# ScissorJack-ever/AlayaLite

Hardware: AMD Instinct MI355X
Metric: QPS @ recall@10>=0.95, GIST-960 L2, 1M base / 1k queries (higher is better)
Workload: dtype f32

## Files before the change

alayalite_amd/csrc/capi.cpp:

```cpp
#include "../../include/alaya_hip.h"

#include <hip/hip_runtime_api.h>

#include <algorithm>
#include <cfloat>
#include <cmath>
#include <cstring>
#include <memory>
#include <mutex>
#include <stdexcept>
#include <limits>
#include <string>
#include <thread>
#include <vector>

#include "build_kernels.h"
#include "extend_kernels.h"
#include "graph_update.h"
#include "hnsw_build.h"
#include "flat_bound.h"
#include "flat_filtered_kernels.h"
#include "flat_kernels.h"
#include <cstdlib>
#include "screen_bound.h"
// ... 93 lines not shown
  bool norms_ready = false;
  DevBuf flat_tiles, tiles_cand, tiles_qexp;
  bool tiles_ready = false;
  int tiles_exp = 0;
  int tiles_metric = -1;
  float max_norm = 0.f;
  DevBuf work, overflow, dirty, stab, q_buf, id_buf, dist_buf, cnt_buf, dlist_buf, dout_buf;
  DevBuf allow_buf, group_buf;
  DevBuf through_buf;
  DevBuf ff_ids, ff_sums, ff_count, ff_part_d, ff_part_i, ff_qlist;
  uint64_t ff_last[4] = {0, 0, 0, 0};
  size_t overflow_clean = 0;
  size_t stab_clean = 0;
  uint32_t hash_log2_override = 0;
  int helpers_mode = -1;
  DevBuf help_stats;
  uint64_t help_stats_slots = 0;
  struct ScreenCopy {
    DevBuf rows, err;
    uint64_t cap = 0;
    bool ready = false;
    bool failed = false;
  };
  ScreenCopy screen_copy[2];
  uint32_t screen_format = 0;
  DevBuf screen_stats;
  uint64_t screen_stats_slots = 0;
  uint32_t last_grid = 0, last_waves = 0;
  uint32_t last_lds = 0, last_hash_log2 = 0, last_compact = 0, last_per_cu = 0, last_scout = 0;
  DevBuf scout_stats;
  uint64_t scout_stats_slots = 0;
  DevBuf scout_policy_stats;
  uint32_t last_scout_policy = 0;
  int visited_mode_override = 0;
  int num_cus = 0;
  uint64_t capacity = 0;
  std::unique_ptr<alaya_amd::HostGraph> upd_graph;
  std::unique_ptr<alaya_amd::RowMirror> upd_rows;
  std::unique_ptr<alaya_amd::UpdateContext> upd_ctx;
  hipStream_t stream = nullptr;
  hipEvent_t scratch_ev = nullptr;
  hipStream_t scratch_stream = nullptr;
  bool scratch_used = false;
  uint64_t device_bytes() const {
    return base.bytes + valid.bytes + l0.bytes + levels.bytes + upper_off.bytes +
           upper_edges.bytes + eps.bytes + overflow.bytes + dirty.bytes + stab.bytes + codes.bytes + sq_min.bytes +
           sq_max.bytes;
  }
};

namespace {

void set_device(const alaya_index *ix) { hip_check(hipSetDevice(ix->device), "hipSetDevice"); }

void scratch_acquire(alaya_index *ix, hipStream_t s) {
  if (ix->scratch_used && ix->scratch_stream != s)
    hip_check(hipStreamWaitEvent(s, ix->scratch_ev, 0), "hipStreamWaitEvent");
}
void scratch_release(alaya_index *ix, hipStream_t s) {
  hip_check(hipEventRecord(ix->scratch_ev, s), "hipEventRecord");
  ix->scratch_stream = s;
  ix->scratch_used = true;
}
void scratch_suspect(alaya_index *ix) {
  ix->overflow_clean = 0;
  ix->stab_clean = 0;
// ... 225 lines not shown

struct SearchPlan {
  const alaya_amd::SearchVariant *variant;
  int W;
  size_t lds;
  int grid;
  int per_cu;
};

uint32_t scout_default(uint32_t dim) { return (dim == 768 || dim == 960) ? alaya_amd::kScoutOn : 0u; }

uint32_t scout_requested(uint32_t dim) {
  const char *e = std::getenv("ALAYA_SEARCH_SCOUT");
  const int asked = e && e[0] ? std::atoi(e) : -1;
  uint32_t f = asked < 0 ? scout_default(dim) : (asked == 1 ? alaya_amd::kScoutOn : (asked == 2 ? alaya_amd::kScoutOn | alaya_amd::kScoutVerify : 0u));
  if (f != 0u) {
    const char *m = std::getenv("ALAYA_SEARCH_SCOUT_MISS");
    if (m && std::atoi(m) != 0) f |= alaya_amd::kScoutMiss;
  }
  return f;
}

uint32_t scout_policy_default(uint32_t dim) {
  return (dim == 768 || dim == 960) ? (alaya_amd::kScoutEarly | alaya_amd::kScoutRecheck) : 0u;
}

uint32_t scout_policy_requested(uint32_t dim) {
  const char *e = std::getenv("ALAYA_SEARCH_SCOUT_POLICY");
  if (!(e && e[0])) return scout_policy_default(dim);
  return static_cast<uint32_t>(std::strtoul(e, nullptr, 0)) &
         (alaya_amd::kScoutEarly | alaya_amd::kScoutRecheck);
}

SearchPlan plan_search(alaya_index *ix, SearchParams &p, alaya_amd::SearchRequest r, uint64_t nq, uint32_t ef,
                       hipStream_t stream) {
  using namespace alaya_amd;
  SearchPlan plan{};
  for (;;) {
    plan.variant = &resolve_search_variant(r);
    const int mode = plan.variant->mode;
    if ((r.want & kModeStamp) != 0 && (mode & kModeStamp) == 0)
      throw ArgError("no stamped search kernel for dim " + std::to_string(ix->dim) +
                     (p.sq8_order ? " SQ8 (order " + std::to_string(p.sq8_order) + ")" : std::string(" f32")) +
                     ": see the variant list in search_variants.h");
    p.help = (mode & kModeHelp) != 0;
    p.two_waves = (mode & kModeTwoWaves) != 0;
    p.screen = (mode & kModeScreen) != 0 ? ix->screen_format : 0u;
    plan.W = p.help ? 4 : search_waves(p);
    while (!p.help && plan.W > 1 && static_cast<uint64_t>(plan.W) > nq) plan.W /= 2;
    p.hash_log2 = size_visited(ix, p, *plan.variant, nq, ef, plan.W);
    const bool compact = p.vis_rbits != kVisWide;
    p.wave_lds = static_cast<uint32_t>(search_wave_lds_bytes(ix->stride, ef, p.hash_log2, compact, p.sq8_order));
    bool fits = true;
    if (p.help) {
      const size_t need = static_cast<size_t>(plan.W) * kHelpMemoSlots * ix->R * 8;
      const size_t q_bytes = search_query_lds_bytes(ix->stride, p.sq8_order);
      if (q_bytes >= need) {
        p.memo_off = 0;
      } else if (p.wave_lds >= q_bytes + 3 * 64 * 4 + need) {
        p.memo_off = static_cast<uint32_t>(q_bytes + 3 * 64 * 4);
      } else {
        fits = false;
      }
    }
    plan.lds = search_shared_lds_bytes(ix->stride, p.sq8_order != 0) + static_cast<size_t>(plan.W) * p.wave_lds +
               (p.help ? kHelpBoardBytes : 0);
    if (!p.help || (fits && plan.lds <= kLdsPerCu)) break;
    r.want &= ~kModeHelp;
  }
  if (plan.lds > kLdsPerCu) throw ArgError("ef / dim too large for the LDS budget");
  int per_cu = 0;
  hip_check(search_occupancy(*plan.variant, p.ip, plan.W, plan.lds, &per_cu), "occupancy");
  per_cu = static_cast<int>(std::max<uint64_t>(1, std::min<uint64_t>(per_cu, max_search_waves_per_cu() / plan.W)));
  const uint64_t cus = static_cast<uint64_t>(stream_cus(ix, stream));
  const uint64_t blocks_needed = p.help ? static_cast<uint64_t>(per_cu) * cus : (nq + plan.W - 1) / plan.W;
  plan.grid = static_cast<int>(std::max<uint64_t>(1, std::min<uint64_t>(blocks_needed, static_cast<uint64_t>(per_cu) * cus)));
  plan.per_cu = per_cu;
  p.scout = 0u;
  p.scout_policy = 0u;
  const uint32_t scout = scout_requested(ix->dim);
  if (scout != 0u && p.screen == 3u && !p.ip && !p.two_waves && !p.help && plan.W == 1 && ix->R <= kScoutR &&
      (plan.variant->mode & ~kModeScreen) == 0 && search_has_two_waves(ix->dim, p.sq8_order, ix->generic) &&
      !helpers_requested(ix, p, nq, cus)) {
    SearchRequest r2 = r;
    r2.want |= kModeTwoWaves;
    const SearchVariant &v2 = resolve_search_variant(r2);
    const size_t lds2 = plan.lds + kScoutBoardBytes;
    int per_cu2 = 0;
    if (v2.mode == (kModeScreen | kModeTwoWaves) && lds2 <= kLdsPerCu)
      hip_check(search_occupancy(v2, false, 2, lds2, &per_cu2), "occupancy");
    if (per_cu2 >= per_cu && nq <= static_cast<uint64_t>(per_cu) * cus) {
      plan.variant = &v2;
      plan.lds = lds2;
      p.scout = scout;
      p.scout_policy = scout_policy_requested(ix->dim);
      if (const char *e = std::getenv("ALAYA_SEARCH_SCOUT_GRID"))
        plan.grid = std::max(1, std::min(plan.grid, std::atoi(e)));
    }
  }
  return plan;
}

SearchParams graph_search_params(alaya_index *ix, const float *d_q, uint64_t nq, uint32_t k, uint32_t ef, uint32_t *d_ids,
                                 float *d_dists, uint32_t *d_cnt) {
  SearchParams p = base_params(ix);
  p.l0 = ix->l0.as<uint32_t>();
  p.R = ix->R;
  p.dedup_edges = ix->dedup;
  p.levels = ix->has_overlay ? ix->levels.as<uint32_t>() : nullptr;
  p.upper_off = ix->upper_off.as<uint64_t>();
  p.upper_edges = ix->upper_edges.as<uint32_t>();
  p.upper_R = ix->upper_R;
  p.ep = ix->ep;
  p.eps = ix->eps.as<uint32_t>();
  p.n_eps = ix->n_eps;
  p.queries = d_q;
  p.nq = nq;
  p.q_stride = ix->dim;
  p.k = k;
  p.ef = ef;
  p.out_ids = d_ids;
  p.out_dists = d_dists;
  p.out_counters = d_cnt;
  return p;
}

void set_search_space(alaya_index *ix, SearchParams &p, bool sq8, uint32_t ef) {
  if (sq8) {
    p.sq8_order = ix->sq8_order;
    p.codes = ix->codes.as<uint8_t>();
    p.code_stride = ix->code_stride;
    p.sq_min = ix->sq_min.as<float>();
    p.sq_max = ix->sq_max.as<float>();
  }
  p.stab_log2 = spill_table_log2(p.sq8_order, std::max<uint32_t>(1, ceil_log2(std::max<uint64_t>(ix->n, 2))), ef);
}

void record_launch(alaya_index *ix, SearchParams &p, int grid, int wg_waves, size_t lds, int per_cu, uint64_t searchers,
                   hipStream_t stream) {
  ix->last_grid = static_cast<uint32_t>(grid);
  ix->last_waves = static_cast<uint32_t>(wg_waves);
  ix->last_lds = static_cast<uint32_t>(lds);
  ix->last_hash_log2 = p.hash_log2;
  ix->last_compact = p.vis_rbits != alaya_amd::kVisWide ? 1u : 0u;
  ix->last_per_cu = static_cast<uint32_t>(per_cu);
  ix->last_scout = p.scout;
  ix->last_scout_policy = p.scout_policy;
  ix->scout_stats_slots = p.scout ? searchers : 0;
  ix->help_stats_slots = p.help ? searchers : 0;
  ix->screen_stats_slots = p.screen ? searchers : 0;
  ix->work.reserve(4);
  p.work_counter = ix->work.as<uint32_t>();
  hip_check(hipMemsetAsync(p.work_counter, 0, 4, stream), "hipMemsetAsync");
}

void do_search(alaya_index *ix, const float *d_q, uint64_t nq, uint32_t k, uint32_t ef,
               uint32_t *d_ids, float *d_dists, uint32_t *d_cnt, hipStream_t stream,
               uint64_t *d_stamps = nullptr, bool sq8 = false, uint32_t fill_id = 0) {
  if (!ix->base.ptr) throw ArgError("index has no base vectors");
  if (!ix->has_graph) throw ArgError("index has no graph");
  if (ef == 0) throw ArgError("ef must be >= 1");
  if (k == 0 || nq == 0) return;
  if (ix->graph_n > ix->n) throw ArgError("graph has more nodes than base vectors");
  SearchParams p = graph_search_params(ix, d_q, nq, k, ef, d_ids, d_dists, d_cnt);
  p.stamps = d_stamps;
  p.fill_id = fill_id;
  if (sq8 && !ix->has_sq8) throw ArgError("index has no SQ8 codes");
  set_search_space(ix, p, sq8, ef);
  if (const char *e = std::getenv("ALAYA_HELP_FLAGS")) p.help_flags = static_cast<uint32_t>(std::strtoul(e, nullptr, 10));
  const SearchPlan plan = plan_search(ix, p, search_request(ix, p, nq, ef, stream), nq, ef, stream);
  if (p.screen >= 2) {
    p.screen_u8 = ix->screen_copy[1].rows.as<uint8_t>();
  } else if (p.screen) {
    p.screen_rows = ix->screen_copy[0].rows.as<uint16_t>();
    p.screen_err = ix->screen_copy[0].err.as<float>();
  }
  scratch_acquire(ix, stream);
  const uint64_t searchers = static_cast<uint64_t>(plan.grid) * plan.W;
  prepare_spill(ix, p, searchers, stream);
  const int wg_waves = p.scout ? 2 * plan.W : plan.W;
  if (p.scout) {
    ix->scout_stats.reserve(searchers * 16);
    p.scout_stats = ix->scout_stats.as<uint32_t>();
    ix->scout_policy_stats.reserve(searchers * 12);
    p.scout_policy_stats = ix->scout_policy_stats.as<uint32_t>();
  }
// ... 1982 lines not shown
    hipStream_t s = nullptr;
    hip_check(hipExtStreamCreateWithCUMask(&s, static_cast<uint32_t>(mask.size()), mask.data()),
              "hipExtStreamCreateWithCUMask");
    *stream = s;
  });
}

int alaya_stream_destroy(void *stream) {
  return guarded([&] {
    if (stream) hip_check(hipStreamDestroy(static_cast<hipStream_t>(stream)), "hipStreamDestroy");
  });
}

int alaya_index_last_launch(const alaya_index *ix, uint32_t *workgroups, uint32_t *waves_per_group) {
  return guarded([&] {
    if (!ix) throw ArgError("null index");
    if (workgroups) *workgroups = ix->last_grid;
    if (waves_per_group) *waves_per_group = ix->last_waves;
  });
}

int alaya_index_last_plan(const alaya_index *ix, uint32_t *lds_bytes, uint32_t *hash_log2, uint32_t *compact,
                          uint32_t *groups_per_cu, uint32_t *scout) {
  return guarded([&] {
    if (!ix) throw ArgError("null index");
    if (lds_bytes) *lds_bytes = ix->last_lds;
    if (hash_log2) *hash_log2 = ix->last_hash_log2;
    if (compact) *compact = ix->last_compact;
    if (groups_per_cu) *groups_per_cu = ix->last_per_cu;
    if (scout) *scout = ix->last_scout;
  });
}

static std::vector<uint64_t> searcher_stats(alaya_index *ix, const DevBuf &buf, uint64_t searchers, uint32_t words) {
  std::vector<uint64_t> t(words, 0);
  if (searchers) {
    set_device(ix);
    scratch_drain(ix);
    std::vector<uint32_t> h(words * searchers);
    hip_check(hipMemcpy(h.data(), buf.ptr, h.size() * 4, hipMemcpyDeviceToHost), "D2H");
    for (uint64_t i = 0; i < h.size(); ++i) t[i % words] += h[i];
  }
  return t;
}

int alaya_index_scout_stats(alaya_index *ix, uint64_t *expansions, uint64_t *hits, uint64_t *records,
                            uint64_t *mismatches) {
  return guarded_scratch(ix, [&] {
    if (!ix) throw ArgError("null index");
    const std::vector<uint64_t> t = searcher_stats(ix, ix->scout_stats, ix->scout_stats_slots, 4);
    if (expansions) *expansions = t[0];
    if (hits) *hits = t[1];
    if (records) *records = t[2];
    if (mismatches) *mismatches = t[3];
  });
}

int alaya_index_scout_policy_stats(alaya_index *ix, uint32_t *policy, uint64_t *early_posts, uint64_t *confirmed,
                                   uint64_t *abandoned) {
  return guarded_scratch(ix, [&] {
    if (!ix) throw ArgError("null index");
    const bool sums = early_posts || confirmed || abandoned;
    const std::vector<uint64_t> t = searcher_stats(ix, ix->scout_policy_stats, sums ? ix->scout_stats_slots : 0, 3);
    if (policy) *policy = ix->last_scout_policy;
    if (early_posts) *early_posts = t[0];
    if (confirmed) *confirmed = t[1];
    if (abandoned) *abandoned = t[2];
  });
}

int alaya_index_set_helpers(alaya_index *ix, int mode) {
  return guarded([&] {
    if (!ix) throw ArgError("null index");
    if (mode < -1 || mode > 1) throw ArgError("helpers mode must be -1 (automatic), 0 (off) or 1 (on)");
    ix->helpers_mode = mode;
  });
}

int alaya_index_help_stats(alaya_index *ix, uint64_t *memo_dists, uint64_t *memo_expansions, uint64_t *helper_rows) {
  return guarded_scratch(ix, [&] {
    if (!ix) throw ArgError("null index");
    const std::vector<uint64_t> t = searcher_stats(ix, ix->help_stats, ix->help_stats_slots, 3);
    if (memo_dists) *memo_dists = t[0];
    if (memo_expansions) *memo_expansions = t[1];
    if (helper_rows) *helper_rows = t[2];
  });
}

int alaya_screen_lower_bound(const float *d_tilde, const float *e_row, uint64_t n, uint32_t dim, float *out) {
  return guarded([&] {
    if (n && (!d_tilde || !e_row || !out)) throw ArgError("invalid arguments");
    for (uint64_t i = 0; i < n; ++i) out[i] = alaya_amd::screen_lower_bound(d_tilde[i], e_row[i], dim);
  });
}

namespace {
void screen_u8_quantize_one(const float *x, uint32_t dim, uint8_t *codes, float *header, float *values) {
  using namespace alaya_amd;
  float lo = FLT_MAX, hi = -FLT_MAX;
  bool bad = false;
// ... 138 lines not shown
```

alayalite_amd/csrc/pybind_module.cpp:

```cpp
#include <pybind11/numpy.h>
#include <pybind11/pybind11.h>
#include <pybind11/stl.h>

#include <algorithm>
#include <cmath>
#include <cstring>
#include <fstream>
#include <memory>
#include <queue>
#include <stdexcept>
#include <string>
#include <vector>

#include "../../include/alaya_hip.h"

extern "C" int alaya_index_flat_diag(alaya_index *, const float *, uint64_t, uint32_t, int, uint32_t *, float *,
                                     uint32_t *, uint32_t *, void *);
#include "host_distance.h"

namespace py = pybind11;

namespace alaya_py {

enum class IndexType { FLAT = 0, HNSW = 1, NSG = 2, FUSION = 3, QG = 4 };
// ... 112 lines not shown
  void set_hash_log2(uint32_t v) { check(alaya_index_set_hash_log2(ix_, v)); }
  void set_visited_mode(int m) { check(alaya_index_set_visited_mode(ix_, m)); }
  void set_helpers(int m) { check(alaya_index_set_helpers(ix_, m)); }
  py::tuple last_launch() {
    uint32_t g = 0, w = 0;
    check(alaya_index_last_launch(ix_, &g, &w));
    return py::make_tuple(g, w);
  }
  py::tuple help_stats() {
    uint64_t m = 0, x = 0, r = 0;
    check(alaya_index_help_stats(ix_, &m, &x, &r));
    return py::make_tuple(m, x, r);
  }
  py::tuple screen_stats() {
    uint64_t a = 0, b = 0;
    check(alaya_index_screen_stats(ix_, &a, &b));
    return py::make_tuple(a, b);
  }
  py::tuple scout_stats() {
    uint64_t e = 0, h = 0, r = 0, m = 0;
    check(alaya_index_scout_stats(ix_, &e, &h, &r, &m));
    return py::make_tuple(e, h, r, m);
  }
  py::tuple scout_policy_stats() {
    uint64_t a = 0, c = 0, d = 0;
    check(alaya_index_scout_policy_stats(ix_, nullptr, &a, &c, &d));
    return py::make_tuple(a, c, d);
  }
  uint32_t scout_policy() {
    uint32_t pol = 0;
    check(alaya_index_scout_policy_stats(ix_, &pol, nullptr, nullptr, nullptr));
    return pol;
  }
  py::dict last_plan() {
    uint32_t g = 0, w = 0, lds = 0, hl = 0, c = 0, pc = 0, sc = 0;
    check(alaya_index_last_launch(ix_, &g, &w));
    check(alaya_index_last_plan(ix_, &lds, &hl, &c, &pc, &sc));
    py::dict d;
    d["workgroups"] = g;
    d["waves_per_group"] = w;
    d["lds_bytes"] = lds;
    d["hash_log2"] = hl;
    d["compact"] = c != 0;
    d["groups_per_cu"] = pc;
    d["scout"] = sc;
    d["scout_policy"] = scout_policy();
    return d;
  }

 protected:
  alaya_index *ix_ = nullptr;
};

class PyIndexInterface : public LaunchControls {
 public:
  explicit PyIndexInterface(const IndexParams &params) : params_(params) {
    dtype_ = dtype_code(params_.data_type_);
    if (params_.id_type_.is(py::dtype::of<uint32_t>())) {
      id_bytes_ = 4;
    } else if (params_.id_type_.is(py::dtype::of<uint64_t>())) {
      id_bytes_ = 8;
    } else {
      throw std::runtime_error("Unsupported id type");
    }
    if (params_.quantization_type_ == QuantizationType::SQ4 ||
        params_.quantization_type_ == QuantizationType::RABITQ)
      throw std::runtime_error("quantization type not supported by the MI355X engine (SQ4/RaBitQ are out of scope)");
    if (params_.metric_ == MetricType::COS && dtype_ != kF32 && dtype_ != kF64) {
      throw std::runtime_error("COS metric only support float or double");
    }
    if (params_.quantization_type_ == QuantizationType::SQ8 && dtype_ != kF32)
      throw std::runtime_error("SQ8 quantization of non-float32 data is not supported by the MI355X engine");
    check(alaya_index_create(0, &ix_));
  }
  ~PyIndexInterface() {
    if (graph_) alaya_graph_free(graph_);
    if (ix_) alaya_index_destroy(ix_);
  }
  PyIndexInterface(const PyIndexInterface &) = delete;
// ... 958 lines not shown
      .def("get_data_by_id", &PyIndexInterface::get_data_by_id, py::arg("id"))
      .def("insert", &PyIndexInterface::insert, py::arg("insert_data"), py::arg("ef"))
      .def("remove", &PyIndexInterface::remove, py::arg("id"))
      .def("add", &PyIndexInterface::add, py::arg("vectors"), py::arg("ef_construction"))
      .def("sq8_codes", &PyIndexInterface::sq8_codes)
      .def("sq8_range", &PyIndexInterface::sq8_range)
      .def("last_build_device_ms", &PyIndexInterface::last_build_device_ms)
      .def("batch_search", &PyIndexInterface::batch_search, py::arg("queries"), py::arg("topk"),
           py::arg("ef"), py::arg("num_threads"))
      .def("batch_search_with_distance", &PyIndexInterface::batch_search_with_distance,
           py::arg("queries"), py::arg("topk"), py::arg("ef"), py::arg("num_threads"))
      .def("exact_search", &PyIndexInterface::exact_search, py::arg("queries"), py::arg("topk"))
      .def("exact_search_filtered", &PyIndexInterface::exact_search_filtered, py::arg("queries"), py::arg("topk"),
           py::arg("allow_words"), py::arg("mask_of_query") = py::none())
      .def("save", &PyIndexInterface::save, py::arg("index_path"), py::arg("data_path"),
           py::arg("quant_path") = std::string())
      .def("load", &PyIndexInterface::load, py::arg("index_path"), py::arg("data_path"),
           py::arg("quant_path") = std::string())
      .def("filtered_search", &PyIndexInterface::filtered_search, py::arg("queries"), py::arg("topk"), py::arg("ef"),
           py::arg("allow_words"), py::arg("mask_of_query") = py::none(), py::arg("pool") = 0,
           py::arg("through") = false)
      .def("last_through", &PyIndexInterface::last_through)
      .def("get_data_dim", &PyIndexInterface::get_data_dim)
      .def("get_data_num", &PyIndexInterface::get_data_num)
      .def("last_counters", &PyIndexInterface::last_counters)
      .def("set_hash_log2", &PyIndexInterface::set_hash_log2)
      .def("set_visited_mode", &PyIndexInterface::set_visited_mode)
      .def("set_helpers", &PyIndexInterface::set_helpers)
      .def("last_launch", &PyIndexInterface::last_launch)
      .def("help_stats", &PyIndexInterface::help_stats)
      .def("screen_stats", &PyIndexInterface::screen_stats)
      .def("scout_stats", &PyIndexInterface::scout_stats)
      .def("scout_policy_stats", &PyIndexInterface::scout_policy_stats)
      .def("last_plan", &PyIndexInterface::last_plan)
      .def("set_rerank_mode", &PyIndexInterface::set_rerank_mode)
      .def("rerank_mode", &PyIndexInterface::rerank_mode)
      .def("device_distances", &PyIndexInterface::device_distances)
      .def("graph_arrays", &PyIndexInterface::graph_arrays);


  py::class_<Graph, std::shared_ptr<Graph>>(m, "Graph")
      .def_static("build", &Graph::build, py::arg("data"), py::arg("metric") = 0, py::arg("R") = 32u,
                  py::arg("ef_construction") = 100u, py::arg("num_threads") = 1u, py::arg("seed") = 100u)
      .def_static("load", &Graph::load, py::arg("path"), py::arg("id_bytes") = 4)
      .def_static("from_arrays", &Graph::from_arrays, py::arg("l0"), py::arg("levels"), py::arg("upper_off"),
                  py::arg("upper_edges"), py::arg("upper_R"), py::arg("ep"), py::arg("eps") = py::none())
      .def("save", &Graph::save, py::arg("path"), py::arg("id_bytes") = 4, py::arg("capacity") = 0u)
      .def("arrays", &Graph::arrays);
  py::class_<DeviceIndex, std::shared_ptr<DeviceIndex>>(m, "DeviceIndex")
      .def(py::init<int>(), py::arg("device") = 0)
      .def("set_base", &DeviceIndex::set_base, py::arg("rows"), py::arg("metric") = 0, py::arg("valid") = py::none())
      .def("set_graph", &DeviceIndex::set_graph)
      .def("build_graph", &DeviceIndex::build_graph, py::arg("R") = 32, py::arg("ef_construction") = 100,
           py::arg("seed") = 100, py::arg("batch_div") = 0, py::arg("max_batch") = 0, py::arg("refine") = 2)
      .def("extend_graph", &DeviceIndex::extend_graph, py::arg("rows"), py::arg("ef_construction") = 100,
           py::arg("seed") = 100, py::arg("batch_div") = 0, py::arg("max_batch") = 0, py::arg("refine") = 2)
      .def("read_sq8", &DeviceIndex::read_sq8, py::arg("first"), py::arg("count"))
      .def("search", &DeviceIndex::search, py::arg("queries"), py::arg("k"), py::arg("ef"))
      .def("search_device", &DeviceIndex::search_device)
      .def("filtered_search", &DeviceIndex::filtered_search, py::arg("queries"), py::arg("k"), py::arg("ef"),
           py::arg("allow_words"), py::arg("mask_of_query") = py::none())
      .def("filtered_search_device", &DeviceIndex::filtered_search_device)
      .def("filtered_search_hop", &DeviceIndex::filtered_search_hop, py::arg("queries"), py::arg("k"), py::arg("ef"),
           py::arg("allow_words"), py::arg("mask_of_query") = py::none())
      .def("filtered_search_hop_device", &DeviceIndex::filtered_search_hop_device)
      .def("filtered_search_sq8", &DeviceIndex::filtered_search_sq8, py::arg("queries"), py::arg("k"), py::arg("ef"),
           py::arg("allow_words"), py::arg("mask_of_query") = py::none(), py::arg("pool") = 0,
           py::arg("rerank_queries") = py::none())
      .def("filtered_search_sq8_device", &DeviceIndex::filtered_search_sq8_device)
      .def("shard_search_device", &DeviceIndex::shard_search_device)
      .def("distances", &DeviceIndex::distances)
      .def("set_hash_log2", &DeviceIndex::set_hash_log2)
      .def("set_visited_mode", &DeviceIndex::set_visited_mode)
      .def("set_helpers", &DeviceIndex::set_helpers)
      .def("last_launch", &DeviceIndex::last_launch)
      .def("help_stats", &DeviceIndex::help_stats)
      .def("screen_stats", &DeviceIndex::screen_stats)
      .def("scout_stats", &DeviceIndex::scout_stats)
      .def("scout_policy_stats", &DeviceIndex::scout_policy_stats)
      .def("last_plan", &DeviceIndex::last_plan)
      .def("flat_search", &DeviceIndex::flat_search, py::arg("queries"), py::arg("k"))
      .def("flat_search_device", &DeviceIndex::flat_search_device)
      .def("flat_search_filtered", &DeviceIndex::flat_search_filtered, py::arg("queries"), py::arg("k"),
           py::arg("allow_words"), py::arg("mask_of_query") = py::none())
      .def("flat_search_filtered_device", &DeviceIndex::flat_search_filtered_device)
      .def("flat_filtered_last", &DeviceIndex::flat_filtered_last)
      .def("flat_diag", &DeviceIndex::flat_diag)
      .def("flat_contraction", &DeviceIndex::flat_contraction)
      .def("search_sq8_device", &DeviceIndex::search_sq8_device)
      .def("shard_search_sq8_device", &DeviceIndex::shard_search_sq8_device)
      .def("set_sq8", &DeviceIndex::set_sq8, py::arg("codes"), py::arg("min"), py::arg("max"), py::arg("order") = 2)
      .def("search_sq8", &DeviceIndex::search_sq8, py::arg("queries"), py::arg("k"), py::arg("ef"),
           py::arg("rerank") = 1, py::arg("rerank_queries") = py::none())
      .def("profile_search", &DeviceIndex::profile_search, py::arg("q"), py::arg("k"), py::arg("ef"),
           py::arg("space") = 0)
      .def("device_bytes", &DeviceIndex::device_bytes);
  m.def("sq8_train", [](F32Array data) {
    const uint32_t d = static_cast<uint32_t>(data.shape(1));
    py::array_t<float> mn(d), mx(d);
    check(alaya_sq8_train(data.data(), data.shape(0), d, mn.mutable_data(), mx.mutable_data()));
    return py::make_tuple(mn, mx);
  });
  m.def("sq8_encode", [](F32Array data, F32Array mn, F32Array mx, uint32_t threads) {
    py::array_t<uint8_t> codes({data.shape(0), data.shape(1)});
    check(alaya_sq8_encode(data.data(), data.shape(0), static_cast<uint32_t>(data.shape(1)), mn.data(), mx.data(),
                           codes.mutable_data(), threads));
    return codes;
  }, py::arg("data"), py::arg("min"), py::arg("max"), py::arg("num_threads") = 1u);
  m.def("host_sq8_order", &host_sq8_order);
  m.def("build_batches", [](U32Array levels, uint64_t start, uint32_t ep, uint32_t batch_div, uint32_t max_batch) {
    if (levels.ndim() != 1) throw py::value_error("levels must be 1D");
    const uint64_t n = levels.shape(0);
// ... 97 lines not shown
```

alayalite_amd/csrc/search_kernels.h:

```cpp
#pragma once
#include <hip/hip_runtime_api.h>

#include <cstddef>
#include <cstdint>

#include "search_variants.h"

namespace alaya_amd {

struct SearchParams {
  const float *base;
  uint64_t n;
  uint32_t dim;
  uint32_t stride;
  const uint32_t *valid;
  bool ip;
  bool generic;
  const uint32_t *l0;
  uint32_t R;
  bool dedup_edges;
  const uint32_t *levels;
  const uint64_t *upper_off;
  const uint32_t *upper_edges;
  uint32_t upper_R;
// ... 13 lines not shown
  uint32_t *overflow_bits;
  uint32_t *dirty_words;
  uint32_t dirty_cap;
  uint32_t wave_lds;
  uint32_t hash_log2;
  uint32_t vis_rbits;
  uint32_t vis_lbits;
  uint32_t vis_max_disp;
  uint32_t vis_limit;
  uint16_t *spill_table;
  uint32_t stab_log2;
  uint32_t stab_rbits;
  uint32_t spill_flags;
  uint64_t *stamps;
  int sq8_order;
  const uint8_t *codes;
  uint32_t code_stride;
  const float *sq_min;
  const float *sq_max;
  uint32_t help;
  uint32_t help_flags;
  uint32_t memo_off;
  uint32_t two_waves;
  uint32_t *help_stats;
  uint32_t screen;
  const uint16_t *screen_rows;
  const float *screen_err;
  const uint8_t *screen_u8;
  uint32_t *screen_stats;
  uint32_t scout;
  uint32_t *scout_stats;
  uint32_t scout_policy;
  uint32_t *scout_policy_stats;
};
constexpr uint32_t kScoutOn = 1, kScoutVerify = 2, kScoutMiss = 4;
constexpr uint32_t kScoutEarly = 1, kScoutRecheck = 2;
constexpr uint32_t kScoutSlots = 3;
constexpr uint32_t kScoutR = 32;
constexpr size_t kScoutBoardBytes = kScoutSlots * (kScoutR * 4 + 8 + 4) + 20;

struct FilterParams {
  const uint32_t *allow;
  const uint32_t *mask_of_query;
  uint32_t mask_words;
  uint32_t k;
  uint32_t result_off;
};

struct HopParams {
  uint32_t *n_through;
};

struct RerankParams {
  const uint32_t *search_ids;
  uint32_t k;
  uint32_t n_src;
  uint32_t n_take;
  uint32_t zeros;
  uint32_t fill_id;
  uint32_t *out_ids;
  float *out_dists;
};

constexpr uint32_t kVisWide = 0xffffffffu;
constexpr size_t kHelpBoardBytes = 256;
#ifndef ALAYA_HELP_DEPTH
#define ALAYA_HELP_DEPTH 1
#endif
constexpr size_t kHelpMemoSlots = ALAYA_HELP_DEPTH + 1;
constexpr uint32_t kStabBucket = 8;
inline size_t visited_table_bytes(uint32_t hash_log2, bool compact) {
// ... 35 lines not shown
```

alayalite_amd/csrc/search_kernels.hip:

```cpp
#include <hip/hip_runtime.h>

#include <cfloat>
#include <cstdint>

#include "screen_bound.h"
#include "search_kernels.h"
#include "search_device.h"

#ifndef ALAYA_MIN_WAVES_SQ8
#define ALAYA_MIN_WAVES_SQ8 -1
#endif
#ifndef ALAYA_MIN_WAVES_NARROW
#define ALAYA_MIN_WAVES_NARROW 0
#endif
#ifndef ALAYA_MIN_WAVES_WIDE
#define ALAYA_MIN_WAVES_WIDE 0
#endif
template <int kSpace>
constexpr bool space_sq8() { return kSpace == 1 || kSpace == 2; }
template <int kSpace>
constexpr bool space_tab() { return kSpace == 2; }

template <int kChunks, int kSpace, int kMode = 0>
constexpr int search_min_waves() {
// ... 430 lines not shown
      const uint32_t v = adjacency_row(p, static_cast<int>(R), node);
      const uint32_t cnt = static_cast<uint32_t>(adjacency_count(static_cast<int>(R), v));
      if (pos >= cnt) {
        if (lane == 0) exhausted[t * kHelpSlots + s] = seq;
        wave_sync();
        continue;
      }
      worked = true;
      const Lds Lt = carve_lds<kSpace>(p, smem, t);
      bool want = static_cast<uint32_t>(lane) >= pos && static_cast<uint32_t>(lane) < min(pos + kHelpClaim, cnt);
      if (hint) want = want && !sibling_visited<kSpace>(p, Lt, t, v, want);
      const uint64_t wm = ballot(want);
      const int n = __popcll(wm);
      if (n == 0) continue;
      const uint32_t slot = __popcll(wm & ((1ull << lane) - 1ull));
      if (want) L.cid[slot] = v;
      wave_sync();
      space_distances<kIP, kChunks, kSpace>(p, Lt, L.cid, n, L.cd);
      if (lane == 0) b->own[wave].rows += static_cast<uint32_t>(n);
      if (want) {
        const uint64_t e = (static_cast<uint64_t>(seq) << 32) | __float_as_uint(L.cd[slot]);
        __hip_atomic_store(memo + (static_cast<uint32_t>(t) * kHelpSlots + s) * R + lane, e, __ATOMIC_RELAXED,
                           __HIP_MEMORY_SCOPE_WORKGROUP);
      }
      wave_sync();
    }
    if (!worked) __builtin_amdgcn_s_sleep(4);
  }
}

constexpr uint32_t kScoutDone = 0xffffffffu;
constexpr uint32_t kScoutMissing = 0xffffffffu;
constexpr uint64_t kScoutNoMatch = 1ull << 63;
struct ScoutBoard {
  uint64_t tag[kScoutSlots];
  uint32_t bound[kScoutSlots][kScoutR];
  uint32_t req[kScoutSlots];
  uint32_t state;
  uint32_t stat[3];
  uint32_t early;
};
static_assert(sizeof(ScoutBoard) == kScoutBoardBytes && kScoutSlots == 3, "board size");

__device__ __forceinline__ ScoutBoard *scout_board(const SearchParams &p, unsigned char *smem, int n_search, int i) {
  return reinterpret_cast<ScoutBoard *>(smem + search_shared_lds_bytes(p.stride, p.sq8_order != 0) +
                                        static_cast<size_t>(n_search) * p.wave_lds) + i;
}

template <typename T>
__device__ __forceinline__ T lds_load(const T *a) {
  return __hip_atomic_load(a, __ATOMIC_RELAXED, __HIP_MEMORY_SCOPE_WORKGROUP);
}
template <typename T, typename U>
__device__ __forceinline__ void lds_store(T *a, U v) {
  __hip_atomic_store(a, static_cast<T>(v), __ATOMIC_RELAXED, __HIP_MEMORY_SCOPE_WORKGROUP);
}
__device__ __forceinline__ void lds_order() { asm volatile("" ::: "memory"); }

__device__ __forceinline__ uint64_t scout_key(uint32_t epoch, uint32_t node) {
  return (static_cast<uint64_t>(epoch & 0x7fffffffu) << 32) | node;
}

__device__ __forceinline__ void scout_post(ScoutBoard *b, int first, int n, uint32_t x0, uint32_t x1, uint32_t x2) {
  const int lane = lane_id();
  if (lane < n) lds_store(&b->req[first + lane], lane == 0 ? x0 : (lane == 1 ? x1 : x2));
}

__device__ __forceinline__ void scout_board_init(ScoutBoard *b) {
  const int lane = lane_id();
  if (lane < static_cast<int>(kScoutSlots)) {
    b->req[lane] = kEmpty;
    b->tag[lane] = 0ull;
    b->stat[lane] = 0u;
    b->state = 0u;
    b->early = 0u;
  }
}

__device__ __forceinline__ void scout_query_end(ScoutBoard *b) {
  if (lane_id() == 0) lds_store(&b->state, 0u);
  lds_order();
  scout_post(b, 0, 3, kEmpty, kEmpty, kEmpty);
}

__device__ __forceinline__ void scout_query_begin(ScoutBoard *b, uint32_t epoch) {
  lds_order();
  if (lane_id() == 0) lds_store(&b->state, epoch);
}

__device__ __forceinline__ bool scout_lookup(ScoutBoard *b, uint32_t epoch, uint32_t u, bool fresh, uint32_t slot, float *cd) {
  const int lane = lane_id();
  bool memo_ok = false;
  const uint64_t key = scout_key(epoch, u);
  uint64_t tg = 0ull;
  if (lane < static_cast<int>(kScoutSlots)) tg = lds_load(&b->tag[lane]);
  const uint64_t rows = ballot(tg == key);
  if (rows != 0ull) {
    const int row = __ffsll(static_cast<unsigned long long>(rows)) - 1;
    lds_order();
    const uint32_t mb = lds_load(&b->bound[row][lane & static_cast<int>(kScoutR - 1)]);
    lds_order();
    const uint64_t again = lds_load(&b->tag[row]);
    memo_ok = ballot(again != key || (fresh && (mb == kScoutMissing || lane >= static_cast<int>(kScoutR)))) == 0ull;
    if (memo_ok && fresh) cd[slot] = __uint_as_float(mb);
  }
  if (lane == 0) lds_store(&b->req[0], kEmpty);
  return memo_ok;
}

__device__ __forceinline__ void scout_count_screen(ScoutBoard *b, bool hit) {
  if (lane_id() == 0) {
    b->stat[0] += 1u;
    if (hit) b->stat[1] += 1u;
  }
}

__device__ __forceinline__ void scout_early_request(ScoutBoard *b, const Lds &L, const PoolState &ps, bool keep, float lb3,
                                                    uint32_t c, uint32_t pred) {
  const uint32_t kb = keep ? (lb3 > 0.f ? __float_as_uint(lb3) : 0u) : 0xffffffffu;
  uint32_t mn = min(kb, lane_xor<1>(kb));
  mn = min(mn, lane_xor<2>(mn));
  mn = min(mn, lane_xor<4>(mn));
  mn = min(mn, lane_xor<8>(mn));
  mn = min(mn, lane_xor<16>(mn));
  mn = min(read_lane(mn, 0), read_lane(mn, 32));
  if (__uint_as_float(mn) < L.pd[ps.cur]) {
    const uint32_t cand = read_lane(c, __ffsll(static_cast<unsigned long long>(ballot(kb == mn))) - 1);
    scout_post(b, 1, 2, cand, pred, kEmpty);
    if (lane_id() == 0 && (b->early & 0xffffu) != 0xffffu) b->early += 1u;
  }
}

__device__ __forceinline__ void scout_count_mismatches(ScoutBoard *b, uint32_t bad, int lane) {
  if (lane == 0 && bad != 0u) b->stat[2] += bad;
}

__device__ __forceinline__ void scout_retarget(ScoutBoard *b, bool early, uint32_t nx, uint32_t old_pred) {
// ... 53 lines not shown
    if (read_lane(lds_load(&b->state), 0) != sq_epoch) continue;
    const uint32_t u = read_lane(rq, 0), c1 = read_lane(rq, 1), c2 = read_lane(rq, 2);
    const uint64_t ku = scout_key(e, u), k1 = scout_key(e, c1), k2 = scout_key(e, c2);
    tg &= ~kScoutNoMatch;
    const bool have1 = ballot(tg == k1) != 0ull, have2 = ballot(tg == k2) != 0ull;
    uint32_t node = kEmpty;
    if (!miss && c1 != kEmpty && !have1) {
      node = c1;
    } else if (c2 != kEmpty && !have2) {
      node = c2;
    }
    const uint64_t spare = ballot(lane < static_cast<int>(kScoutSlots) && tg != ku && tg != k1 && tg != k2);
    if (node == kEmpty || spare == 0ull) {
      __builtin_amdgcn_s_sleep(8);
      continue;
    }
    const int row = __ffsll(static_cast<unsigned long long>(spare)) - 1;
    const uint32_t v = adjacency_row(p, R, node);
    const int cnt = adjacency_count(R, v);
    bool want = lane < cnt;
    want = want && !sibling_visited<0>(p, Ls, 0, v, want);
    const uint64_t wm = ballot(want);
    if (recheck) {
      lds_order();
      uint32_t rq2 = kEmpty;
      if (lane < static_cast<int>(kScoutSlots)) rq2 = lds_load(&b->req[lane]);
      lds_order();
      const uint32_t e2 = read_lane(lds_load(&b->state), 0);
      if (e2 != e || (read_lane(rq2, 1) != node && read_lane(rq2, 2) != node)) {
        ++abandoned;
        continue;
      }
    }
    if (lane == 0) lds_store(&b->tag[row], 0ull);
    lds_order();
    uint32_t lb_bits = kScoutMissing;
    if (wm != 0ull) {
      const uint32_t v0 = read_lane(v, __ffsll(static_cast<unsigned long long>(wm)) - 1);
      const uint32_t id = want ? v : v0;
      const uint32_t idm = static_cast<uint32_t>(__builtin_amdgcn_ds_bpermute(mine << 2, static_cast<int>(id)));
      const uint8_t *rp = p.screen_u8 + static_cast<uint64_t>(idm) * rec;
      const float4 head = *reinterpret_cast<const float4 *>(rp);
      const uint2 sums = *reinterpret_cast<const uint2 *>(rp + screen_u8_sums_offset(p.stride));
      const uint32_t ac = screen_dots_pass<kChunks>(p, sq.codes, id, NoHook());
      const float lb = screen_int_bound(p.stride, sq.err, sq.lo, sq.scale, sq.a1, sq.a2, head.x, head.y, head.z, sums.x,
                                        sums.y, ac);
      if ((wm >> mine) & 1ull) lb_bits = __float_as_uint(lb);
      records += static_cast<uint32_t>(__popcll(wm));
    }
    if (lane < 32 && mine < R) lds_store(&b->bound[row][mine], lb_bits);
    lds_order();
    if (lane == 0) lds_store(&b->tag[row], scout_key(e, node) | (miss ? kScoutNoMatch : 0ull));
  }
  if (stats != nullptr && lane == 0) stats[2] = records;
  if (policy_stats != nullptr && lane == 0) policy_stats[2] = abandoned;
}

__device__ __forceinline__ void screen_stats_out(const SearchParams &p, uint64_t slot, uint32_t n_screened,
                                                 uint32_t n_screened_out, int lane) {
  if (p.screen_stats != nullptr && lane == 0) {
    p.screen_stats[2 * slot] = n_screened;
    p.screen_stats[2 * slot + 1] = n_screened_out;
  }
}

template <bool kIP, int kChunks, int kMode, int kSpace = 0>
__global__ void __launch_bounds__(256)
// ... 138 lines not shown
      }
      if (!vs.spilled && vs.count + 64 > vs.limit) spill_begin<space_tab<kSpace>()>(vs);
      if constexpr (kCheck && space_tab<kSpace>()) {
        if (u == pre_u && vs.spilled && vs.stab != nullptr) {
          stab_order();
          uint32_t home, code;
          stab_key(vs, v, home, code);
          uint64_t lo2 = 0ull, hi2 = 0ull;
          if (act) stab_load(vs, home, lo2, hi2);
          if (ballot(act && (lo2 != pre_lo || hi2 != pre_hi))) n_hops_up |= 0x40000000u;
        }
      }
      const bool fresh = visit<space_tab<kSpace>()>(vs, v, act, kSpillPrefetch && u == pre_u, pre_lo, pre_hi);
      if constexpr (kSpillPrefetch) {
        __builtin_amdgcn_sched_barrier(0);
        asm volatile("" ::: "memory");
      }
      pre_u = kEmpty;
      pre_lo = pre_hi = 0ull;
      const uint64_t fm = ballot(fresh);
      const int nf = __popcll(fm);
      pred = ps.cur < ps.size ? (L.pi[ps.cur] & kIdMask) : kEmpty;
      if (pred != kEmpty) pred_v = adjacency_row(p, static_cast<int>(p.R), pred, pred_v);
#ifdef ALAYA_FINE_STAMPS
      stamp(5);
#else
      stamp(2);
#endif
      if (nf == 0) continue;
      const uint32_t slot = __popcll(fm & ((1ull << lane) - 1ull));
      if (fresh) L.cid[slot] = v;
      bool memo_ok = false;
      if constexpr (kScout) {
        if (scouting && ps.size == ps.ef && p.screen == 3) memo_ok = scout_lookup(sboard, qi + 1u, u, fresh, slot, L.cd);
      }
      const uint32_t *dist_ids = L.cid;
      bool compute = true;
      if constexpr (kHelp) {
        if (look != 0u) {
          const uint32_t seq = look >> 2;
          const int hs = static_cast<int>(look & 3u);
          const uint64_t *memo = help_memo<kSpace>(p, smem, mine.memo_wave) +
                                 (static_cast<uint32_t>(wave) * kHelpSlots + hs) * p.R;
          uint64_t e = 0ull;
          if (fresh) e = __hip_atomic_load(memo + lane, __ATOMIC_RELAXED, __HIP_MEMORY_SCOPE_WORKGROUP);
          const bool got = fresh && static_cast<uint32_t>(e >> 32) == seq;
          help_retire(board, wave, hs, seq);
          uint32_t *ids2 = reinterpret_cast<uint32_t *>(L.sd);
          if (fresh) {
            ids2[slot] = got ? kEmpty : v;
            if (got) L.cd[slot] = __uint_as_float(static_cast<uint32_t>(e));
          }
          dist_ids = ids2;
          const uint32_t n_got = __popcll(ballot(got));
          help_count(board, wave, n_got, static_cast<uint32_t>(nf), lane);
          compute = n_got < static_cast<uint32_t>(nf);
        }
      }
      wave_sync();
      auto second_level_prefetch = [&]() {
        if constexpr (kSpillPrefetch) {
          if (vs.spilled && pred != kEmpty && !(p.spill_flags & 1u)) {
            if (p.spill_flags & 4u) __builtin_amdgcn_s_waitcnt(0);
            spill_prefetch(vs, pred_v, lane < static_cast<int>(p.R), pre_lo, pre_hi);
            pre_u = pred;
          }
        }
// ... 922 lines not shown
```

include/alaya_hip.h:

```cpp
#ifndef ALAYA_HIP_H_
#define ALAYA_HIP_H_

#include <stddef.h>
#include <stdint.h>

#ifdef __cplusplus
extern "C" {
#endif

#define ALAYA_OK 0
#define ALAYA_ERR_ARG 1
#define ALAYA_ERR_RUNTIME 2
#define ALAYA_ERR_DEVICE 3

#define ALAYA_METRIC_L2 0
#define ALAYA_METRIC_IP 1
#define ALAYA_METRIC_COS 2
#define ALAYA_DIST_GENERIC 0x100

typedef struct alaya_index alaya_index;
typedef struct alaya_graph alaya_graph;

const char *alaya_last_error(void);
const char *alaya_build_info(void);
// ... 103 lines not shown
                                     uint32_t *ids, float *dists);
int alaya_index_flat_search_filtered_device(alaya_index *ix, const float *d_queries, uint64_t nq, uint32_t k,
                                            const uint32_t *d_allow_words, uint32_t n_masks,
                                            const uint32_t *d_mask_of_query, uint32_t *d_ids, float *d_dists,
                                            void *stream);
int alaya_index_flat_filtered_last(const alaya_index *ix, uint64_t *out);
int alaya_flat_filtered_plan(uint64_t n_allowed, uint64_t nq, uint32_t k, uint32_t stride, uint32_t cus,
                             uint64_t *out);
int alaya_index_set_hash_log2(alaya_index *ix, uint32_t log2_slots);
int alaya_index_set_visited_mode(alaya_index *ix, int mode);
int alaya_index_set_helpers(alaya_index *ix, int mode);
int alaya_index_help_stats(alaya_index *ix, uint64_t *memo_dists, uint64_t *memo_expansions,
                           uint64_t *helper_rows);
int alaya_index_screen_stats(alaya_index *ix, uint64_t *screened, uint64_t *screened_out);
int alaya_screen_lower_bound(const float *d_tilde, const float *e_row, uint64_t n, uint32_t dim, float *out);
int alaya_screen_u8_quantize(const float *rows, uint64_t n, uint32_t dim, uint8_t *codes, float *header,
                             float *values);
int alaya_screen_int_bound(const float *queries, const float *rows, uint64_t n, uint32_t dim, float *d_in,
                           float *e_sum, float *bound, uint32_t *sums);
int alaya_flat_ip_slack(int contraction, uint32_t k_acc, const float *q_norm2, const int *q_exp, uint64_t n,
                        float b_max, int base_exp, float *out);
int alaya_flat_ip_proven(const float *kth_d, const float *cutoff, const float *slack, uint64_t n, uint8_t *out);
int alaya_search_variant(uint32_t dim, int ip, int sq8_order, int generic, uint32_t wanted_mode, int *space,
                         uint32_t *chunks, uint32_t *mode, uint32_t *has_mode);
int alaya_search_variant_at(uint32_t index, int *space, uint32_t *chunks, uint32_t *mode, int *l2_only,
                            uint32_t *count);
int alaya_index_last_launch(const alaya_index *ix, uint32_t *workgroups, uint32_t *waves_per_group);
int alaya_index_last_plan(const alaya_index *ix, uint32_t *lds_bytes, uint32_t *hash_log2, uint32_t *compact,
                          uint32_t *groups_per_cu, uint32_t *scout);
int alaya_index_scout_stats(alaya_index *ix, uint64_t *expansions, uint64_t *hits, uint64_t *records,
                            uint64_t *mismatches);
int alaya_index_scout_policy_stats(alaya_index *ix, uint32_t *policy, uint64_t *early_posts, uint64_t *confirmed,
                                   uint64_t *abandoned);
int alaya_index_info(const alaya_index *ix, uint64_t *n, uint32_t *dim, uint32_t *stride,
                     int *metric, uint64_t *device_bytes);

#ifdef __cplusplus
}
#endif
#endif
```

Measured before the change: 357,000.

## Let searcher wait on in-flight scout results instead of recomputing distances

The scout wave now marks a board slot as in flight, with a tag bit, while it computes lower bounds for a node. When the main searcher finds its node in flight, it polls the LDS tag with s_sleep, up to a fixed poll limit, rather than missing and computing the distances itself. This is on by default for dim 960. It also adds per-wave atomic counters in global memory for wait statistics and widens the memset per launch. The intent is to turn late scout results into hits, at the risk of stalling the searcher while it spins and of extra atomic traffic.

```diff
diff --git a/alayalite_amd/csrc/capi.cpp b/alayalite_amd/csrc/capi.cpp
--- a/alayalite_amd/csrc/capi.cpp
+++ b/alayalite_amd/csrc/capi.cpp
@@ -149,6 +149,7 @@
   uint64_t scout_stats_slots = 0;
   DevBuf scout_policy_stats;
   uint32_t last_scout_policy = 0;
+  uint32_t last_scout_wait = 0;
   int visited_mode_override = 0;
   int num_cus = 0;
   uint64_t capacity = 0;
@@ -440,6 +441,16 @@
          (alaya_amd::kScoutEarly | alaya_amd::kScoutRecheck);
 }
 
+uint32_t scout_wait_default(uint32_t dim) { return dim == 960 ? 1u : 0u; }
+
+constexpr size_t kScoutWaitOffset = 256;
+
+uint32_t scout_wait_requested(uint32_t dim) {
+  const char *e = std::getenv("ALAYA_SEARCH_SCOUT_WAIT");
+  if (!(e && e[0])) return scout_wait_default(dim);
+  return std::atoi(e) != 0 ? 1u : 0u;
+}
+
 SearchPlan plan_search(alaya_index *ix, SearchParams &p, alaya_amd::SearchRequest r, uint64_t nq, uint32_t ef,
                        hipStream_t stream) {
   using namespace alaya_amd;
@@ -486,6 +497,7 @@
   plan.per_cu = per_cu;
   p.scout = 0u;
   p.scout_policy = 0u;
+  p.scout_wait = 0u;
   const uint32_t scout = scout_requested(ix->dim);
   if (scout != 0u && p.screen == 3u && !p.ip && !p.two_waves && !p.help && plan.W == 1 && ix->R <= kScoutR &&
       (plan.variant->mode & ~kModeScreen) == 0 && search_has_two_waves(ix->dim, p.sq8_order, ix->generic) &&
@@ -502,6 +514,7 @@
       plan.lds = lds2;
       p.scout = scout;
       p.scout_policy = scout_policy_requested(ix->dim);
+      p.scout_wait = (scout & kScoutMiss) != 0u ? 0u : scout_wait_requested(ix->dim);
       if (const char *e = std::getenv("ALAYA_SEARCH_SCOUT_GRID"))
         plan.grid = std::max(1, std::min(plan.grid, std::atoi(e)));
     }
@@ -554,12 +567,15 @@
   ix->last_per_cu = static_cast<uint32_t>(per_cu);
   ix->last_scout = p.scout;
   ix->last_scout_policy = p.scout_policy;
+  ix->last_scout_wait = p.scout_wait;
   ix->scout_stats_slots = p.scout ? searchers : 0;
   ix->help_stats_slots = p.help ? searchers : 0;
   ix->screen_stats_slots = p.screen ? searchers : 0;
-  ix->work.reserve(4);
+  const size_t wait_bytes = p.scout ? kScoutWaitOffset + searchers * alaya_amd::kScoutWaitWords * 4 : 0;
+  ix->work.reserve(std::max<size_t>(4, wait_bytes));
   p.work_counter = ix->work.as<uint32_t>();
-  hip_check(hipMemsetAsync(p.work_counter, 0, 4, stream), "hipMemsetAsync");
+  p.scout_wait_stats = p.scout ? p.work_counter + kScoutWaitOffset / 4 : nullptr;
+  hip_check(hipMemsetAsync(p.work_counter, 0, std::max<size_t>(4, wait_bytes), stream), "hipMemsetAsync");
 }
 
 void do_search(alaya_index *ix, const float *d_q, uint64_t nq, uint32_t k, uint32_t ef,
@@ -2608,13 +2624,14 @@
   });
 }
 
-static std::vector<uint64_t> searcher_stats(alaya_index *ix, const DevBuf &buf, uint64_t searchers, uint32_t words) {
+static std::vector<uint64_t> searcher_stats(alaya_index *ix, const DevBuf &buf, uint64_t searchers, uint32_t words,
+                                            size_t offset = 0) {
   std::vector<uint64_t> t(words, 0);
   if (searchers) {
     set_device(ix);
     scratch_drain(ix);
     std::vector<uint32_t> h(words * searchers);
-    hip_check(hipMemcpy(h.data(), buf.ptr, h.size() * 4, hipMemcpyDeviceToHost), "D2H");
+    hip_check(hipMemcpy(h.data(), static_cast<const char *>(buf.ptr) + offset, h.size() * 4, hipMemcpyDeviceToHost), "D2H");
     for (uint64_t i = 0; i < h.size(); ++i) t[i % words] += h[i];
   }
   return t;
@@ -2642,6 +2659,23 @@
     if (early_posts) *early_posts = t[0];
     if (confirmed) *confirmed = t[1];
     if (abandoned) *abandoned = t[2];
+  });
+}
+
+int alaya_index_scout_wait_stats(alaya_index *ix, uint32_t *wait, uint64_t *in_flight_seen, uint64_t *late_hits,
+                                 uint64_t *gave_up, uint64_t *polls, uint64_t *late_by_polls) {
+  return guarded_scratch(ix, [&] {
+    if (!ix) throw ArgError("null index");
+    const bool sums = in_flight_seen || late_hits || gave_up || polls || late_by_polls;
+    const std::vector<uint64_t> t =
+        searcher_stats(ix, ix->work, sums ? ix->scout_stats_slots : 0, alaya_amd::kScoutWaitWords, kScoutWaitOffset);
+    if (wait) *wait = ix->last_scout_wait;
+    if (in_flight_seen) *in_flight_seen = t[0];
+    if (late_hits) *late_hits = t[1];
+    if (gave_up) *gave_up = t[2];
+    if (polls) *polls = t[3];
+    if (late_by_polls)
+      for (int i = 0; i < 4; ++i) late_by_polls[i] = t[4 + i];
   });
 }
 
diff --git a/alayalite_amd/csrc/pybind_module.cpp b/alayalite_amd/csrc/pybind_module.cpp
--- a/alayalite_amd/csrc/pybind_module.cpp
+++ b/alayalite_amd/csrc/pybind_module.cpp
@@ -168,6 +168,21 @@
     check(alaya_index_scout_policy_stats(ix_, &pol, nullptr, nullptr, nullptr));
     return pol;
   }
+  py::tuple scout_wait_stats() {
+    uint64_t s = 0, l = 0, g = 0;
+    check(alaya_index_scout_wait_stats(ix_, nullptr, &s, &l, &g, nullptr, nullptr));
+    return py::make_tuple(s, l, g);
+  }
+  py::tuple scout_wait_polls() {
+    uint64_t p = 0, h[4] = {0, 0, 0, 0};
+    check(alaya_index_scout_wait_stats(ix_, nullptr, nullptr, nullptr, nullptr, &p, h));
+    return py::make_tuple(p, h[0], h[1], h[2], h[3]);
+  }
+  uint32_t scout_wait() {
+    uint32_t w = 0;
+    check(alaya_index_scout_wait_stats(ix_, &w, nullptr, nullptr, nullptr, nullptr, nullptr));
+    return w;
+  }
   py::dict last_plan() {
     uint32_t g = 0, w = 0, lds = 0, hl = 0, c = 0, pc = 0, sc = 0;
     check(alaya_index_last_launch(ix_, &g, &w));
@@ -181,6 +196,7 @@
     d["groups_per_cu"] = pc;
     d["scout"] = sc;
     d["scout_policy"] = scout_policy();
+    d["scout_wait"] = scout_wait();
     return d;
   }
 
@@ -1205,6 +1221,8 @@
       .def("screen_stats", &PyIndexInterface::screen_stats)
       .def("scout_stats", &PyIndexInterface::scout_stats)
       .def("scout_policy_stats", &PyIndexInterface::scout_policy_stats)
+      .def("scout_wait_stats", &PyIndexInterface::scout_wait_stats)
+      .def("scout_wait_polls", &PyIndexInterface::scout_wait_polls)
       .def("last_plan", &PyIndexInterface::last_plan)
       .def("set_rerank_mode", &PyIndexInterface::set_rerank_mode)
       .def("rerank_mode", &PyIndexInterface::rerank_mode)
@@ -1251,6 +1269,8 @@
       .def("screen_stats", &DeviceIndex::screen_stats)
       .def("scout_stats", &DeviceIndex::scout_stats)
       .def("scout_policy_stats", &DeviceIndex::scout_policy_stats)
+      .def("scout_wait_stats", &DeviceIndex::scout_wait_stats)
+      .def("scout_wait_polls", &DeviceIndex::scout_wait_polls)
       .def("last_plan", &DeviceIndex::last_plan)
       .def("flat_search", &DeviceIndex::flat_search, py::arg("queries"), py::arg("k"))
       .def("flat_search_device", &DeviceIndex::flat_search_device)
diff --git a/alayalite_amd/csrc/search_kernels.h b/alayalite_amd/csrc/search_kernels.h
--- a/alayalite_amd/csrc/search_kernels.h
+++ b/alayalite_amd/csrc/search_kernels.h
@@ -69,11 +69,15 @@
   uint32_t *scout_stats;
   uint32_t scout_policy;
   uint32_t *scout_policy_stats;
+  uint32_t scout_wait;
+  uint32_t *scout_wait_stats;
 };
 constexpr uint32_t kScoutOn = 1, kScoutVerify = 2, kScoutMiss = 4;
 constexpr uint32_t kScoutEarly = 1, kScoutRecheck = 2;
 constexpr uint32_t kScoutSlots = 3;
 constexpr uint32_t kScoutR = 32;
+constexpr uint32_t kScoutWaitWords = 8;
+constexpr uint32_t kScoutWaitPolls = 1024;
 constexpr size_t kScoutBoardBytes = kScoutSlots * (kScoutR * 4 + 8 + 4) + 20;
 
 struct FilterParams {
diff --git a/alayalite_amd/csrc/search_kernels.hip b/alayalite_amd/csrc/search_kernels.hip
--- a/alayalite_amd/csrc/search_kernels.hip
+++ b/alayalite_amd/csrc/search_kernels.hip
@@ -486,6 +486,7 @@
 constexpr uint32_t kScoutDone = 0xffffffffu;
 constexpr uint32_t kScoutMissing = 0xffffffffu;
 constexpr uint64_t kScoutNoMatch = 1ull << 63;
+constexpr uint64_t kScoutInFlight = 1ull << 62;
 struct ScoutBoard {
   uint64_t tag[kScoutSlots];
   uint32_t bound[kScoutSlots][kScoutR];
@@ -512,7 +513,7 @@
 __device__ __forceinline__ void lds_order() { asm volatile("" ::: "memory"); }
 
 __device__ __forceinline__ uint64_t scout_key(uint32_t epoch, uint32_t node) {
-  return (static_cast<uint64_t>(epoch & 0x7fffffffu) << 32) | node;
+  return (static_cast<uint64_t>(epoch & 0x3fffffffu) << 32) | node;
 }
 
 __device__ __forceinline__ void scout_post(ScoutBoard *b, int first, int n, uint32_t x0, uint32_t x1, uint32_t x2) {
@@ -542,13 +543,35 @@
   if (lane_id() == 0) lds_store(&b->state, epoch);
 }
 
-__device__ __forceinline__ bool scout_lookup(ScoutBoard *b, uint32_t epoch, uint32_t u, bool fresh, uint32_t slot, float *cd) {
+__device__ __forceinline__ void scout_wait_count(uint32_t *w, uint32_t n) {
+  (void)__hip_atomic_fetch_add(w, n, __ATOMIC_RELAXED, __HIP_MEMORY_SCOPE_AGENT);
+}
+
+__device__ __forceinline__ bool scout_lookup(ScoutBoard *b, uint32_t epoch, uint32_t u, bool fresh, uint32_t slot, float *cd,
+                                             bool wait, uint32_t *ws) {
   const int lane = lane_id();
   bool memo_ok = false;
   const uint64_t key = scout_key(epoch, u);
   uint64_t tg = 0ull;
   if (lane < static_cast<int>(kScoutSlots)) tg = lds_load(&b->tag[lane]);
-  const uint64_t rows = ballot(tg == key);
+  uint64_t rows = ballot(tg == key);
+  uint32_t polls = 0u;
+  if (rows == 0ull) {
+    const uint64_t flying = ballot(tg == (key | kScoutInFlight));
+    if (flying != 0ull) {
+      if (lane == 0) scout_wait_count(ws, 1u);
+      if (wait) {
+        const int row = __ffsll(static_cast<unsigned long long>(flying)) - 1;
+        uint64_t t;
+        do {
+          __builtin_amdgcn_s_sleep(2);
+          t = lds_load(&b->tag[row]);
+          ++polls;
+        } while (ballot(t == (key | kScoutInFlight)) != 0ull && polls < kScoutWaitPolls);
+        if (ballot(t == key) != 0ull) rows = 1ull << row;
+      }
+    }
+  }
   if (rows != 0ull) {
     const int row = __ffsll(static_cast<unsigned long long>(rows)) - 1;
     lds_order();
@@ -557,6 +580,11 @@
     const uint64_t again = lds_load(&b->tag[row]);
     memo_ok = ballot(again != key || (fresh && (mb == kScoutMissing || lane >= static_cast<int>(kScoutR)))) == 0ull;
     if (memo_ok && fresh) cd[slot] = __uint_as_float(mb);
+  }
+  if (polls != 0u && lane < 3) {
+    const uint32_t len = polls < 8u ? 0u : (polls < 32u ? 1u : (polls < 128u ? 2u : 3u));
+    const uint32_t word = lane == 0 ? (memo_ok ? 1u : 2u) : (lane == 1 ? 3u : 4u + len);
+    scout_wait_count(ws + word, lane == 1 ? polls : (lane == 2 && !memo_ok ? 0u : 1u));
   }
   if (lane == 0) lds_store(&b->req[0], kEmpty);
   return memo_ok;
@@ -676,7 +704,7 @@
         continue;
       }
     }
-    if (lane == 0) lds_store(&b->tag[row], 0ull);
+    if (lane == 0) lds_store(&b->tag[row], miss ? 0ull : (scout_key(e, node) | kScoutInFlight));
     lds_order();
     uint32_t lb_bits = kScoutMissing;
     if (wm != 0ull) {
@@ -881,7 +909,9 @@
       if (fresh) L.cid[slot] = v;
       bool memo_ok = false;
       if constexpr (kScout) {
-        if (scouting && ps.size == ps.ef && p.screen == 3) memo_ok = scout_lookup(sboard, qi + 1u, u, fresh, slot, L.cd);
+        if (scouting && ps.size == ps.ef && p.screen == 3)
+          memo_ok = scout_lookup(sboard, qi + 1u, u, fresh, slot, L.cd, p.scout_wait != 0u,
+                                 p.scout_wait_stats + kScoutWaitWords * (static_cast<uint64_t>(blockIdx.x) * W + wave));
       }
       const uint32_t *dist_ids = L.cid;
       bool compute = true;
diff --git a/include/alaya_hip.h b/include/alaya_hip.h
--- a/include/alaya_hip.h
+++ b/include/alaya_hip.h
@@ -159,6 +159,8 @@
                             uint64_t *mismatches);
 int alaya_index_scout_policy_stats(alaya_index *ix, uint32_t *policy, uint64_t *early_posts, uint64_t *confirmed,
                                    uint64_t *abandoned);
+int alaya_index_scout_wait_stats(alaya_index *ix, uint32_t *wait, uint64_t *in_flight_seen, uint64_t *late_hits,
+                                 uint64_t *gave_up, uint64_t *polls, uint64_t *late_by_polls);
 int alaya_index_info(const alaya_index *ix, uint64_t *n, uint32_t *dim, uint32_t *stride,
                      int *metric, uint64_t *device_bytes);
 
```

After: 362,600 (median of 6 runs). 1.02x the previous value.
